# xxlong0/NeuralUDF

Hardware: NVIDIA H100
Metric: ray-samples/sec (render_core fwd+bwd) (higher is better)
Workload: dtype f32

## Files before the change

### neuraludf_b200/csrc/gemm_tc.cuh

```cuda
#pragma once
#include <cuda.h>
#include <cudaTypedefs.h>
#include <cuda_bf16.h>

#include "gemm_simt.cuh"

namespace nudf {
namespace tc {

constexpr int BM = 128;
constexpr int BN = 128;
constexpr int BK = 64;
constexpr int THREADS = 256;
constexpr int A_HALF_BYTES = BM * BK * 2;
constexpr int B_HALF_BYTES = BN * BK * 2;
__host__ __device__ constexpr int b_plane_bytes(int wn) { return wn * BK * 2; }
__host__ __device__ constexpr int acc_ld(int wn) { return wn + 4; }

__host__ __device__ inline int pad16(int n) { return (n + 15) & ~15; }
__host__ __device__ inline int pad64(int k) { return (k + 63) & ~63; }

__host__ __device__ inline uint32_t sw128(uint32_t row, uint32_t k) {
  return (row >> 3) * 1024u + (row & 7u) * 128u + ((((k >> 3) ^ (row & 7u)) & 7u) << 4) + ((k & 7u) << 1);
}

constexpr int TN_PS = 32;
constexpr int TN_RING = 4;
constexpr uint32_t TN_F32_OPND = TN_PS * BM * 4;
constexpr uint32_t TN_F32_STAGE = 2 * TN_F32_OPND;
constexpr uint32_t TN_PLANE = BM * TN_PS * 2;
constexpr uint32_t TN_PLANE_STAGE = 4 * TN_PLANE;
struct TnMaps { CUtensorMap a, b; };
__host__ __device__ inline uint32_t sw128_mn(uint32_t mn, uint32_t k) {
  return (mn >> 6) * 4096u + (k >> 3) * 1024u + (k & 7u) * 128u + ((((mn >> 3) ^ k) & 7u) << 4) + ((mn & 7u) << 1);
}

constexpr uint32_t W_SLOT = BM * BK * 4;
static_assert(W_SLOT == 2 * A_HALF_BYTES, "a slot holds exactly the two bf16 planes of its slice");
__host__ __device__ constexpr int w_ring(int wn) { return wn == 256 ? 3 : 4; }

__device__ __forceinline__ uint32_t pack_bf16(float a, float b) {
  __nv_bfloat162 v = __floats2bfloat162_rn(a, b);
  return *reinterpret_cast<uint32_t*>(&v);
}
template <int NP>
__device__ __forceinline__ void split4(const float x[4], uint2 planes[NP]) {
  float r[4] = {x[0], x[1], x[2], x[3]};
#pragma unroll
  for (int p = 0; p < NP; ++p) {
    float h[4];
#pragma unroll
    for (int j = 0; j < 4; ++j) {
      h[j] = __bfloat162float(__float2bfloat16_rn(r[j]));
      r[j] -= h[j];
    }
    planes[p] = make_uint2(pack_bf16(h[0], h[1]), pack_bf16(h[2], h[3]));
  }
}
__host__ __device__ inline int nt_of(int np) { return np == 2 ? 256 : 128; }
__host__ __device__ inline int n_tiles(int N, int np) { return (N + nt_of(np) - 1) / nt_of(np); }
__host__ __device__ inline int tile_rows(int N, int t, int np) { int r = N - nt_of(np) * t; return pad16(r < nt_of(np) ? r : nt_of(np)); }
__host__ __device__ inline int64_t tile_elems(int N, int K, int t, int np) { return (int64_t)(pad64(K) / 64) * np * tile_rows(N, t, np) * 64; }
__host__ __device__ inline int64_t tile_offset(int N, int K, int t, int np) {
  int64_t o = 0;
  for (int i = 0; i < t; ++i) o += tile_elems(N, K, i, np);
  return o;
}
__host__ __device__ inline int64_t image_elems(int N, int K, int np) { return tile_offset(N, K, n_tiles(N, np), np); }

static __device__ __forceinline__ void tc_prep_weights_body(const float* __restrict__ W, int64_t ldw, int N, int K, int transposed, int np,
                                                            uint16_t* __restrict__ img, int64_t start, int64_t stride) {
  const int Kp = pad64(K);
  const int nt = n_tiles(N, np);
  int64_t total = 0;
  for (int t = 0; t < nt; ++t) total += (int64_t)tile_rows(N, t, np) * Kp;
  for (int64_t idx = start; idx < total; idx += stride) {
    int64_t rem = idx;
    int t = 0;
    while (rem >= (int64_t)tile_rows(N, t, np) * Kp) { rem -= (int64_t)tile_rows(N, t, np) * Kp; ++t; }
    const int rows = tile_rows(N, t, np);
    const int nl = (int)(rem / Kp), k = (int)(rem - (int64_t)nl * Kp);
    const int n = t * nt_of(np) + nl;
    float x = 0.f;
    if (n < N && k < K) x = transposed ? W[(int64_t)k * ldw + n] : W[(int64_t)n * ldw + k];
    const int s = k >> 6, kl = k & 63;
    uint16_t* base = img + tile_offset(N, K, t, np) + (int64_t)s * np * rows * 64;
    const uint32_t off = sw128((uint32_t)nl, (uint32_t)kl) >> 1;
    float r = x;
    for (int p = 0; p < np; ++p) {
      __nv_bfloat16 h = __float2bfloat16_rn(r);
      base[(int64_t)p * rows * 64 + off] = __bfloat16_as_ushort(h);
      r -= __bfloat162float(h);
    }
  }
}
static __global__ void tc_prep_weights_kernel(const float* __restrict__ W, int64_t ldw, int N, int K, int transposed, int np,
                                              uint16_t* __restrict__ img) {
  tc_prep_weights_body(W, ldw, N, K, transposed, np, img, (int64_t)blockIdx.x * blockDim.x + threadIdx.x, (int64_t)gridDim.x * blockDim.x);
}


__device__ __forceinline__ uint32_t smem_u32(const void* p) { return (uint32_t)__cvta_generic_to_shared(p); }
__device__ __forceinline__ uint8_t* align1024(uint8_t* p) {
  return reinterpret_cast<uint8_t*>((reinterpret_cast<uintptr_t>(p) + 1023) & ~(uintptr_t)1023);
}

__device__ __forceinline__ void mbar_init(uint64_t* bar, uint32_t count) {
  asm volatile("mbarrier.init.shared::cta.b64 [%0], %1;" ::"r"(smem_u32(bar)), "r"(count) : "memory");
}
__device__ __forceinline__ void mbar_arrive_expect_tx(uint64_t* bar, uint32_t bytes) {
  asm volatile("mbarrier.arrive.expect_tx.shared::cta.b64 _, [%0], %1;" ::"r"(smem_u32(bar)), "r"(bytes) : "memory");
}
__device__ __forceinline__ uint32_t mbar_try_wait(uint32_t addr, uint32_t parity) {
  uint32_t ok;
  asm volatile(
      "{\n"
      ".reg .pred p;\n"
      "mbarrier.try_wait.parity.shared::cta.b64 p, [%1], %2;\n"
      "selp.u32 %0, 1, 0, p;\n"
      "}\n"
      : "=r"(ok)
      : "r"(addr), "r"(parity)
      : "memory");
  return ok;
}
__device__ __forceinline__ void mbar_wait(uint64_t* bar, uint32_t parity) {
  const uint32_t addr = smem_u32(bar);
  while (!mbar_try_wait(addr, parity)) {
  }
}
__device__ __forceinline__ void fence_barrier_init() { asm volatile("fence.mbarrier_init.release.cluster;" ::: "memory"); }
__device__ __forceinline__ void fence_proxy_async() { asm volatile("fence.proxy.async.shared::cta;" ::: "memory"); }

__device__ __forceinline__ void bulk_g2s(void* smem_dst, const void* gmem_src, uint32_t bytes, uint64_t* bar) {
  asm volatile("cp.async.bulk.shared::cluster.global.mbarrier::complete_tx::bytes [%0], [%1], %2, [%3];" ::"r"(smem_u32(smem_dst)),
               "l"(gmem_src), "r"(bytes), "r"(smem_u32(bar))
               : "memory");
}

__device__ __forceinline__ void tma_load_2d(void* smem_dst, const CUtensorMap* map, int c, int k, uint64_t* bar) {
  asm volatile("cp.async.bulk.tensor.2d.shared::cluster.global.mbarrier::complete_tx::bytes [%0], [%1, {%2, %3}], [%4];"
               ::"r"(smem_u32(smem_dst)), "l"(reinterpret_cast<uint64_t>(map)), "r"(c), "r"(k), "r"(smem_u32(bar))
               : "memory");
}

__device__ __forceinline__ uint64_t make_desc(uint32_t smem_addr) {
  return (uint64_t)((smem_addr & 0x3FFFFu) >> 4) | (1ull << 16) | (64ull << 32) | (1ull << 62);
}
__device__ __forceinline__ uint64_t make_desc_mn(uint32_t smem_addr) {
  return (uint64_t)((smem_addr & 0x3FFFFu) >> 4) | ((uint64_t)(4096 >> 4) << 16) | ((uint64_t)(1024 >> 4) << 32) | (1ull << 62);
}
__device__ __forceinline__ void wg_fence() { asm volatile("wgmma.fence.sync.aligned;" ::: "memory"); }
__device__ __forceinline__ void wg_commit() { asm volatile("wgmma.commit_group.sync.aligned;" ::: "memory"); }
__device__ __forceinline__ void wg_wait_all() { asm volatile("wgmma.wait_group.sync.aligned 0;" ::: "memory"); }
__device__ __forceinline__ void wg_wait_but_one() { asm volatile("wgmma.wait_group.sync.aligned 1;" ::: "memory"); }
template <int N>
__device__ __forceinline__ void fence_operand(float (&d)[N]) {
#pragma unroll
  for (int q = 0; q < N; ++q) asm volatile("" : "+f"(d[q])::"memory");
}
__device__ __forceinline__ float unbias_rz(float r) { return fmaf(__uint_as_float(__float_as_uint(r) & 0xff800000u), 0x1p-24f, r); }

template <int MN_MAJOR = 0>
__device__ __forceinline__ void wgmma_128(float (&d)[64], uint64_t da, uint64_t db, uint32_t accumulate) {
  asm volatile(
      "{\n"
      ".reg .pred p;\n"
      "setp.ne.b32 p, %66, 0;\n"
      "wgmma.mma_async.sync.aligned.m64n128k16.f32.bf16.bf16 "
      "{%0, %1, %2, %3, %4, %5, %6, %7, %8, %9, %10, %11, %12, %13, %14, %15, %16, %17, %18, %19, %20, %21, %22, %23, %24, %25, "
      "%26, %27, %28, %29, %30, %31, %32, %33, %34, %35, %36, %37, %38, %39, %40, %41, %42, %43, %44, %45, %46, %47, %48, %49, "
      "%50, %51, %52, %53, %54, %55, %56, %57, %58, %59, %60, %61, %62, %63}, %64, %65, p, 1, 1, %67, %67;\n"
      "}\n"
      : "+f"(d[0]), "+f"(d[1]), "+f"(d[2]), "+f"(d[3]), "+f"(d[4]), "+f"(d[5]), "+f"(d[6]), "+f"(d[7]), "+f"(d[8]), "+f"(d[9]),
        "+f"(d[10]), "+f"(d[11]), "+f"(d[12]), "+f"(d[13]), "+f"(d[14]), "+f"(d[15]), "+f"(d[16]), "+f"(d[17]), "+f"(d[18]),
        "+f"(d[19]), "+f"(d[20]), "+f"(d[21]), "+f"(d[22]), "+f"(d[23]), "+f"(d[24]), "+f"(d[25]), "+f"(d[26]), "+f"(d[27]),
        "+f"(d[28]), "+f"(d[29]), "+f"(d[30]), "+f"(d[31]), "+f"(d[32]), "+f"(d[33]), "+f"(d[34]), "+f"(d[35]), "+f"(d[36]),
        "+f"(d[37]), "+f"(d[38]), "+f"(d[39]), "+f"(d[40]), "+f"(d[41]), "+f"(d[42]), "+f"(d[43]), "+f"(d[44]), "+f"(d[45]),
        "+f"(d[46]), "+f"(d[47]), "+f"(d[48]), "+f"(d[49]), "+f"(d[50]), "+f"(d[51]), "+f"(d[52]), "+f"(d[53]), "+f"(d[54]),
        "+f"(d[55]), "+f"(d[56]), "+f"(d[57]), "+f"(d[58]), "+f"(d[59]), "+f"(d[60]), "+f"(d[61]), "+f"(d[62]), "+f"(d[63])
      : "l"(da), "l"(db), "r"(accumulate), "n"(MN_MAJOR));
}
__device__ __forceinline__ void wgmma_128_fresh(float (&d)[64], uint64_t da, uint64_t db) {
  asm volatile(
      "{\n"
      ".reg .pred p;\n"
      "setp.ne.b32 p, %66, 0;\n"
      "wgmma.mma_async.sync.aligned.m64n128k16.f32.bf16.bf16 "
      "{%0, %1, %2, %3, %4, %5, %6, %7, %8, %9, %10, %11, %12, %13, %14, %15, %16, %17, %18, %19, %20, %21, %22, %23, %24, %25, "
      "%26, %27, %28, %29, %30, %31, %32, %33, %34, %35, %36, %37, %38, %39, %40, %41, %42, %43, %44, %45, %46, %47, %48, %49, "
      "%50, %51, %52, %53, %54, %55, %56, %57, %58, %59, %60, %61, %62, %63}, %64, %65, p, 1, 1, 0, 0;\n"
      "}\n"
      : "=f"(d[0]), "=f"(d[1]), "=f"(d[2]), "=f"(d[3]), "=f"(d[4]), "=f"(d[5]), "=f"(d[6]), "=f"(d[7]), "=f"(d[8]), "=f"(d[9]),
        "=f"(d[10]), "=f"(d[11]), "=f"(d[12]), "=f"(d[13]), "=f"(d[14]), "=f"(d[15]), "=f"(d[16]), "=f"(d[17]), "=f"(d[18]),
        "=f"(d[19]), "=f"(d[20]), "=f"(d[21]), "=f"(d[22]), "=f"(d[23]), "=f"(d[24]), "=f"(d[25]), "=f"(d[26]), "=f"(d[27]),
        "=f"(d[28]), "=f"(d[29]), "=f"(d[30]), "=f"(d[31]), "=f"(d[32]), "=f"(d[33]), "=f"(d[34]), "=f"(d[35]), "=f"(d[36]),
        "=f"(d[37]), "=f"(d[38]), "=f"(d[39]), "=f"(d[40]), "=f"(d[41]), "=f"(d[42]), "=f"(d[43]), "=f"(d[44]), "=f"(d[45]),
        "=f"(d[46]), "=f"(d[47]), "=f"(d[48]), "=f"(d[49]), "=f"(d[50]), "=f"(d[51]), "=f"(d[52]), "=f"(d[53]), "=f"(d[54]),
        "=f"(d[55]), "=f"(d[56]), "=f"(d[57]), "=f"(d[58]), "=f"(d[59]), "=f"(d[60]), "=f"(d[61]), "=f"(d[62]), "=f"(d[63])
      : "l"(da), "l"(db), "r"(0u));
}

__device__ __forceinline__ void wgmma_256(float (&d)[128], uint64_t da, uint64_t db, uint32_t accumulate) {
  asm volatile(
      "{\n"
      ".reg .pred p;\n"
      "setp.ne.b32 p, %130, 0;\n"
      "wgmma.mma_async.sync.aligned.m64n256k16.f32.bf16.bf16 "
      "{%0, %1, %2, %3, %4, %5, %6, %7, %8, %9, %10, %11, %12, %13, %14, %15, %16, %17, %18, %19, %20, %21, %22, %23, %24, "
      "%25, %26, %27, %28, %29, %30, %31, %32, %33, %34, %35, %36, %37, %38, %39, %40, %41, %42, %43, %44, %45, %46, %47, "
      "%48, %49, %50, %51, %52, %53, %54, %55, %56, %57, %58, %59, %60, %61, %62, %63, %64, %65, %66, %67, %68, %69, %70, "
      "%71, %72, %73, %74, %75, %76, %77, %78, %79, %80, %81, %82, %83, %84, %85, %86, %87, %88, %89, %90, %91, %92, %93, "
      "%94, %95, %96, %97, %98, %99, %100, %101, %102, %103, %104, %105, %106, %107, %108, %109, %110, %111, %112, %113, "
      "%114, %115, %116, %117, %118, %119, %120, %121, %122, %123, %124, %125, %126, %127}, %128, %129, p, 1, 1, 0, 0;\n"
      "}\n"
      : "+f"(d[0]), "+f"(d[1]), "+f"(d[2]), "+f"(d[3]), "+f"(d[4]), "+f"(d[5]), "+f"(d[6]), "+f"(d[7]), "+f"(d[8]),
        "+f"(d[9]), "+f"(d[10]), "+f"(d[11]), "+f"(d[12]), "+f"(d[13]), "+f"(d[14]), "+f"(d[15]), "+f"(d[16]), "+f"(d[17]),
        "+f"(d[18]), "+f"(d[19]), "+f"(d[20]), "+f"(d[21]), "+f"(d[22]), "+f"(d[23]), "+f"(d[24]), "+f"(d[25]), "+f"(d[26]),
        "+f"(d[27]), "+f"(d[28]), "+f"(d[29]), "+f"(d[30]), "+f"(d[31]), "+f"(d[32]), "+f"(d[33]), "+f"(d[34]), "+f"(d[35]),
        "+f"(d[36]), "+f"(d[37]), "+f"(d[38]), "+f"(d[39]), "+f"(d[40]), "+f"(d[41]), "+f"(d[42]), "+f"(d[43]), "+f"(d[44]),
        "+f"(d[45]), "+f"(d[46]), "+f"(d[47]), "+f"(d[48]), "+f"(d[49]), "+f"(d[50]), "+f"(d[51]), "+f"(d[52]), "+f"(d[53]),
        "+f"(d[54]), "+f"(d[55]), "+f"(d[56]), "+f"(d[57]), "+f"(d[58]), "+f"(d[59]), "+f"(d[60]), "+f"(d[61]), "+f"(d[62]),
        "+f"(d[63]), "+f"(d[64]), "+f"(d[65]), "+f"(d[66]), "+f"(d[67]), "+f"(d[68]), "+f"(d[69]), "+f"(d[70]), "+f"(d[71]),
        "+f"(d[72]), "+f"(d[73]), "+f"(d[74]), "+f"(d[75]), "+f"(d[76]), "+f"(d[77]), "+f"(d[78]), "+f"(d[79]), "+f"(d[80]),
        "+f"(d[81]), "+f"(d[82]), "+f"(d[83]), "+f"(d[84]), "+f"(d[85]), "+f"(d[86]), "+f"(d[87]), "+f"(d[88]), "+f"(d[89]),
        "+f"(d[90]), "+f"(d[91]), "+f"(d[92]), "+f"(d[93]), "+f"(d[94]), "+f"(d[95]), "+f"(d[96]), "+f"(d[97]), "+f"(d[98]),
        "+f"(d[99]), "+f"(d[100]), "+f"(d[101]), "+f"(d[102]), "+f"(d[103]), "+f"(d[104]), "+f"(d[105]), "+f"(d[106]),
        "+f"(d[107]), "+f"(d[108]), "+f"(d[109]), "+f"(d[110]), "+f"(d[111]), "+f"(d[112]), "+f"(d[113]), "+f"(d[114]),
        "+f"(d[115]), "+f"(d[116]), "+f"(d[117]), "+f"(d[118]), "+f"(d[119]), "+f"(d[120]), "+f"(d[121]), "+f"(d[122]),
        "+f"(d[123]), "+f"(d[124]), "+f"(d[125]), "+f"(d[126]), "+f"(d[127])
      : "l"(da), "l"(db), "r"(accumulate));
}

template <int WN>
__device__ __forceinline__ void wgmma_n(float (&d)[WN / 2], uint64_t da, uint64_t db, uint32_t accumulate) {
  if constexpr (WN == 256) wgmma_256(d, da, db, accumulate);
  else wgmma_128(d, da, db, accumulate);
}
template <int NP, int WN>
__device__ __forceinline__ void mma_slice(float (&d)[WN / 2], uint32_t a, uint32_t a_stride, uint32_t b, uint32_t b_stride, bool zero_first) {
  auto desc = [](uint32_t base, uint32_t stride, int p, int j) { return make_desc(base + p * stride + 32u * j); };
#pragma unroll
  for (int j = 0; j < BK / 16; ++j) {
    const uint32_t acc0 = (zero_first && j == 0) ? 0u : 1u;
    if constexpr (NP == 2) {
      wgmma_n<WN>(d, desc(a, a_stride, 1, j), desc(b, b_stride, 0, j), acc0);
      wgmma_n<WN>(d, desc(a, a_stride, 0, j), desc(b, b_stride, 1, j), 1u);
      wgmma_n<WN>(d, desc(a, a_stride, 0, j), desc(b, b_stride, 0, j), 1u);
    } else {
      wgmma_n<WN>(d, desc(a, a_stride, 2, j), desc(b, b_stride, 0, j), acc0);
      wgmma_n<WN>(d, desc(a, a_stride, 0, j), desc(b, b_stride, 2, j), 1u);
      wgmma_n<WN>(d, desc(a, a_stride, 1, j), desc(b, b_stride, 1, j), 1u);
      wgmma_n<WN>(d, desc(a, a_stride, 1, j), desc(b, b_stride, 0, j), 1u);
      wgmma_n<WN>(d, desc(a, a_stride, 0, j), desc(b, b_stride, 1, j), 1u);
    }
  }
}
__device__ __forceinline__ void mma_slice_mn(float (&d)[64], uint32_t a, uint32_t b, bool zero_first) {
#pragma unroll
  for (int j = 0; j < TN_PS / 16; ++j) {
    const uint32_t acc0 = (zero_first && j == 0) ? 0u : 1u;
    const uint32_t aj = a + 2048u * j, bj = b + 2048u * j;
    wgmma_128<1>(d, make_desc_mn(aj + TN_PLANE), make_desc_mn(bj), acc0);
    wgmma_128<1>(d, make_desc_mn(aj), make_desc_mn(bj + TN_PLANE), 1u);
    wgmma_128<1>(d, make_desc_mn(aj), make_desc_mn(bj), 1u);
  }
}

template <int WN>
__device__ __forceinline__ void acc_to_smem(const float (&d)[WN / 2], float* acc_s, int wg, int wtid) {
  constexpr int LD = acc_ld(WN);
  const int r = 64 * wg + 16 * (wtid >> 5) + ((wtid & 31) >> 2);
  const int c = 2 * (wtid & 3);
#pragma unroll
  for (int g = 0; g < WN / 8; ++g) {
    *reinterpret_cast<float2*>(acc_s + r * LD + 8 * g + c) = make_float2(d[4 * g], d[4 * g + 1]);
    *reinterpret_cast<float2*>(acc_s + (r + 8) * LD + 8 * g + c) = make_float2(d[4 * g + 2], d[4 * g + 3]);
  }
}
template <class Epi> constexpr int epi_rows_in_flight() { return epi_family<Epi>::value == FAM_TC_OTHER ? 2 : 8; }
template <int WN, class Epi>
__device__ __forceinline__ void tile_epilogue(const float* acc_s, int64_t m0, int64_t M, int n0, int n_valid_end, const Epi& epi, int tid) {
  constexpr int LD = acc_ld(WN);
  constexpr int EPI_ROWS = epi_rows_in_flight<Epi>();
  const int cq = tid & 31;
#pragma unroll 1
  for (int h = 0; h < WN / 128; ++h) {
    const int cl = 128 * h + 4 * cq;
    const int col = n0 + cl;
    int nv = n_valid_end - col;
    nv = nv < 4 ? nv : 4;
    if (nv <= 0) break;
    for (int r0 = tid >> 5; r0 < BM; r0 += EPI_ROWS * (THREADS / 32)) {
      typename Epi::Aux aux[EPI_ROWS];
#pragma unroll
      for (int i = 0; i < EPI_ROWS; ++i) {
        const int64_t row = m0 + r0 + i * (THREADS / 32);
        if (row < M) epi.load(row, col, nv, aux[i]);
      }
#pragma unroll
      for (int i = 0; i < EPI_ROWS; ++i) {
        const int r = r0 + i * (THREADS / 32);
        const int64_t row = m0 + r;
        if (row < M) {
          const float4 t = *reinterpret_cast<const float4*>(acc_s + r * LD + cl);
          const float x[4] = {t.x, t.y, t.z, t.w};
          epi.apply(row, col, x, nv, aux[i]);
        }
      }
    }
  }
}

template <int NT>
__device__ __forceinline__ void fetch_a(const float* __restrict__ A, int64_t lda, int64_t m0, int64_t M, int k0, int K, int tid,
                                        bool vec_ok, float4 (&v)[BM * 16 / NT]) {
  const int c = tid & 15;
  const int rsub = tid >> 4;
  const int k = k0 + c * 4;
#pragma unroll
  for (int pass = 0; pass < BM * 16 / NT; ++pass) {
    const int64_t row = m0 + pass * (NT / 16) + rsub;
    v[pass] = make_float4(0.f, 0.f, 0.f, 0.f);
    if (row < M) {
      const float* p = A + row * lda + k;
      if (vec_ok && k + 3 < K) {
        v[pass] = *reinterpret_cast<const float4*>(p);
      } else {
        if (k + 0 < K) v[pass].x = p[0];
        if (k + 1 < K) v[pass].y = p[1];
        if (k + 2 < K) v[pass].z = p[2];
        if (k + 3 < K) v[pass].w = p[3];
      }
    }
  }
}
template <int NP, int NT>
__device__ __forceinline__ void store_a(const float4 (&v)[BM * 16 / NT], uint8_t* sa, int tid) {
  const int c = tid & 15;
  const int rsub = tid >> 4;
#pragma unroll
  for (int pass = 0; pass < BM * 16 / NT; ++pass) {
    const float x[4] = {v[pass].x, v[pass].y, v[pass].z, v[pass].w};
    uint2 pl[NP];
    split4<NP>(x, pl);
    const uint32_t off = sw128((uint32_t)(pass * (NT / 16) + rsub), (uint32_t)(c * 4));
#pragma unroll
    for (int p = 0; p < NP; ++p) *reinterpret_cast<uint2*>(sa + p * A_HALF_BYTES + off) = pl[p];
  }
}
template <int NP, int NT>
__device__ __forceinline__ void stage_a_direct(const float* __restrict__ A, int64_t lda, int64_t m0, int64_t M, int k0, int K,
                                               uint8_t* sa, int tid, bool vec_ok) {
  float4 v[BM * 16 / NT];
  fetch_a<NT>(A, lda, m0, M, k0, K, tid, vec_ok, v);
  store_a<NP, NT>(v, sa, tid);
}

__device__ __forceinline__ void fetch_block_t(const float* __restrict__ X, int64_t ld, int m0, int m_total, int r0, int rows,
                                              int64_t k0, int64_t k_end, int lane, bool vec_ok, float4 (&v)[8][2]) {
  const int mq = lane & 7, kq = lane >> 3;
  if (r0 + 4 * mq >= rows) return;
  const int m = m0 + r0 + 4 * mq;
#pragma unroll
  for (int q = 0; q < 8; ++q) {
#pragma unroll
    for (int kk = 0; kk < 2; ++kk) {
      const int64_t k = k0 + 2 * (4 * q + kq) + kk;
      v[q][kk] = make_float4(0.f, 0.f, 0.f, 0.f);
      if (k < k_end) {
        const float* p = X + k * ld + m;
        if (vec_ok && m + 3 < m_total) {
          v[q][kk] = *reinterpret_cast<const float4*>(p);
        } else {
          if (m + 0 < m_total) v[q][kk].x = p[0];
          if (m + 1 < m_total) v[q][kk].y = p[1];
          if (m + 2 < m_total) v[q][kk].z = p[2];
          if (m + 3 < m_total) v[q][kk].w = p[3];
        }
      }
    }
  }
}
template <bool CSUM = false>
__device__ __forceinline__ void store_block_t(const float4 (&v)[8][2], int r0, int rows, uint8_t* s_hi, uint8_t* s_lo, int lane,
                                              float* csum = nullptr) {
  const int mq = lane & 7, kq = lane >> 3;
  if (r0 + 4 * mq >= rows) return;
  if (CSUM) {
#pragma unroll
    for (int q = 0; q < 8; ++q) {
      csum[0] += v[q][0].x + v[q][1].x; csum[1] += v[q][0].y + v[q][1].y;
      csum[2] += v[q][0].z + v[q][1].z; csum[3] += v[q][0].w + v[q][1].w;
    }
  }
#pragma unroll
  for (int q = 0; q < 8; ++q) {
    const float x0[4] = {v[q][0].x, v[q][0].y, v[q][0].z, v[q][0].w};
    const float x1[4] = {v[q][1].x, v[q][1].y, v[q][1].z, v[q][1].w};
#pragma unroll
    for (int j = 0; j < 4; ++j) {
      const float h0 = __bfloat162float(__float2bfloat16_rn(x0[j])), h1 = __bfloat162float(__float2bfloat16_rn(x1[j]));
      const uint32_t off = sw128((uint32_t)(r0 + 4 * mq + j), (uint32_t)(2 * (4 * q + kq)));
      *reinterpret_cast<uint32_t*>(s_hi + off) = pack_bf16(h0, h1);
      *reinterpret_cast<uint32_t*>(s_lo + off) = pack_bf16(x0[j] - h0, x1[j] - h1);
    }
  }
}

template <int NP, int WN, class Epi, bool RING>
__global__ void __launch_bounds__(THREADS, 1)
gemm_w_kernel(const float* __restrict__ A, int64_t lda, int64_t M, int N, int K, const uint16_t* __restrict__ img, Epi epi,
              const __grid_constant__ CUtensorMap amap) {
  static_assert(WN == 128 || (WN == 256 && NP == 2), "WN = 256 only with 2 planes (3 planes need 2 x WN/2 accumulators)");
  static_assert(!RING || NP == 2, "the ring path splits a slot into 2 planes in place");
  extern __shared__ uint8_t smem_raw[];
  uint8_t* smem = align1024(smem_raw);
  const int tid = threadIdx.x, wg = tid >> 7;
  const int n_ct = (N + WN - 1) / WN;
  const int n0 = (int)(blockIdx.x % (unsigned)n_ct) * WN;
  const int64_t m0 = (int64_t)(blockIdx.x / (unsigned)n_ct) * BM;
  const int t = n0 / nt_of(NP);
  const int rows_t = tile_rows(N, t, NP);
  const int row_in_tile = n0 - t * nt_of(NP);
  int rows_h = rows_t - row_in_tile; rows_h = rows_h < WN ? rows_h : WN;
  const int n_slices = pad64(K) / 64;
  constexpr uint32_t B_PLANE = b_plane_bytes(WN);
  const uint16_t* img_t = img + tile_offset(N, K, t, NP) + (int64_t)row_in_tile * 64;
  constexpr int NACC = WN / 2, NTOT = NP == 3 ? 64 : 1;
  float acc[NACC], tot[NTOT], acc2[NTOT];
#pragma unroll
  for (int q = 0; q < NACC; ++q) acc[q] = 0.f;
#pragma unroll
  for (int q = 0; q < NTOT; ++q) tot[q] = 0.f;

  if constexpr (RING) {
    constexpr int NR = w_ring(WN);
    constexpr uint32_t W_STAGE = 2 * B_PLANE;
    uint8_t* wst = smem + NR * W_SLOT;
    uint64_t* afull = reinterpret_cast<uint64_t*>(wst + 2 * W_STAGE);
    uint64_t* wfull = afull + NR;
    auto issue_a = [&](int i) {
      const int r = i % NR;
      mbar_arrive_expect_tx(&afull[r], W_SLOT);
      tma_load_2d(smem + r * W_SLOT, &amap, i * BK, (int)m0, &afull[r]);
    };
    auto issue_w = [&](int ks) {
      uint8_t* st = wst + (ks & 1) * W_STAGE;
      const uint32_t wb = (uint32_t)rows_h * 128u;
      mbar_arrive_expect_tx(&wfull[ks & 1], 2 * wb);
      for (int p = 0; p < 2; ++p) bulk_g2s(st + p * B_PLANE, img_t + ((int64_t)ks * 2 + p) * rows_t * 64, wb, &wfull[ks & 1]);
    };
    auto split = [&](int i) {
      uint8_t* slot = smem + (i % NR) * W_SLOT;
      mbar_wait(&afull[i % NR], (uint32_t)((i / NR) & 1));
      float4 v[BM * 16 / THREADS];
      const float4* f = reinterpret_cast<const float4*>(slot) + (tid >> 4) * (BK / 4) + (tid & 15);
#pragma unroll
      for (int pass = 0; pass < BM * 16 / THREADS; ++pass) v[pass] = f[pass * (THREADS / 16) * (BK / 4)];
      __syncthreads();
      store_a<2, THREADS>(v, slot, tid);
    };
    if (tid == 0) {
      for (int r = 0; r < NR; ++r) mbar_init(&afull[r], 1);
      mbar_init(&wfull[0], 1);
      mbar_init(&wfull[1], 1);
      fence_barrier_init();
      if (n_slices > 0) issue_w(0);
      for (int i = 0; i < NR && i < n_slices; ++i) issue_a(i);
    }
    __syncthreads();
    if (n_slices > 0) {
      split(0);
      fence_proxy_async();
    }
    __syncthreads();
    for (int ks = 0; ks < n_slices; ++ks) {
      const int s = ks & 1;
      if (tid == 0 && ks + 1 < n_slices) issue_w(ks + 1);
      mbar_wait(&wfull[s], (uint32_t)((ks >> 1) & 1));
      const uint32_t sa = smem_u32(smem + (ks % NR) * W_SLOT), sb = smem_u32(wst + s * W_STAGE);
      wg_fence();
      mma_slice<2, WN>(acc, sa + wg * (64 * 128), A_HALF_BYTES, sb, B_PLANE, ks == 0);
      wg_commit();
      if (ks + 1 < n_slices) split(ks + 1);
      wg_wait_all();
      fence_proxy_async();
      __syncthreads();
      if (tid == 0 && ks + NR < n_slices) issue_a(ks + NR);
    }
  } else {
    const uint32_t a_bytes = NP * A_HALF_BYTES, stage_bytes = a_bytes + NP * B_PLANE;
    uint64_t* full = reinterpret_cast<uint64_t*>(smem + 2 * stage_bytes);
    const bool vec_ok = ((lda & 3) == 0) && aligned16(A);

    auto issue_copies = [&](int ks) {
      uint8_t* st = smem + (ks & 1) * stage_bytes;
      const uint32_t wb = (uint32_t)rows_h * 128u;
      mbar_arrive_expect_tx(&full[ks & 1], NP * wb);
      for (int p = 0; p < NP; ++p) bulk_g2s(st + a_bytes + p * B_PLANE, img_t + ((int64_t)ks * NP + p) * rows_t * 64, wb, &full[ks & 1]);
    };
    if (tid == 0) {
      mbar_init(&full[0], 1);
      mbar_init(&full[1], 1);
      fence_barrier_init();
    }
    __syncthreads();
    if (n_slices > 0) {
      if (tid == 0) issue_copies(0);
      stage_a_direct<NP, THREADS>(A, lda, m0, M, 0, K, smem, tid, vec_ok);
      fence_proxy_async();
    }
    __syncthreads();
    for (int ks = 0; ks < n_slices; ++ks) {
      const int s = ks & 1;
      if (tid == 0 && ks + 1 < n_slices) issue_copies(ks + 1);
      mbar_wait(&full[s], (uint32_t)((ks >> 1) & 1));
      const uint32_t st = smem_u32(smem + s * stage_bytes);
      wg_fence();
      mma_slice<NP, WN>(acc, st + wg * (64 * 128), A_HALF_BYTES, st + a_bytes, B_PLANE, NP == 3 || ks == 0);
      wg_commit();
      if (ks + 1 < n_slices) stage_a_direct<NP, THREADS>(A, lda, m0, M, (ks + 1) * BK, K, smem + (s ^ 1) * stage_bytes, tid, vec_ok);
      wg_wait_all();
      if constexpr (NP == 3) {
        static_assert(BK / 16 == 4, "four hi * hi steps per K slice");
        auto hi_hi = [&](float (&d)[64], int j) {
          wg_fence();
          wgmma_128_fresh(d, make_desc(st + wg * (64 * 128) + 32u * j), make_desc(st + a_bytes + 32u * j));
          wg_commit();
        };
        auto add_unbiased = [&](float (&d)[64]) {
          fence_operand(d);
#pragma unroll
          for (int q = 0; q < 64; ++q) tot[q] += unbias_rz(d[q]);
        };
        hi_hi(acc2, 0);
        fence_operand(acc);
#pragma unroll
        for (int q = 0; q < 64; ++q) tot[q] += acc[q];
        hi_hi(acc, 1);
        wg_wait_but_one();
        add_unbiased(acc2);
        hi_hi(acc2, 2);
        wg_wait_but_one();
        add_unbiased(acc);
        hi_hi(acc, 3);
        wg_wait_but_one();
        add_unbiased(acc2);
        wg_wait_all();
        add_unbiased(acc);
      }
      fence_proxy_async();
      __syncthreads();
    }
  }
  float* acc_s = reinterpret_cast<float*>(smem);
  if constexpr (NP == 3) acc_to_smem<WN>(tot, acc_s, wg, tid & 127);
  else acc_to_smem<WN>(acc, acc_s, wg, tid & 127);
  __syncthreads();
  tile_epilogue<WN>(acc_s, m0, M, n0, N, epi, tid);
}

template <class Epi, bool RING>
__global__ void __launch_bounds__(THREADS, 1)
gemm_tn_kernel(const float* __restrict__ A, int64_t lda, const float* __restrict__ B, int64_t ldb, int M, int N, int64_t K, int64_t k_chunk,
               Epi epi, float* __restrict__ colsum, float* __restrict__ cs_ws, const __grid_constant__ TnMaps maps) {
  extern __shared__ uint8_t smem_raw[];
  uint8_t* smem = align1024(smem_raw);
  const int tid = threadIdx.x, wg = tid >> 7, warp = tid >> 5, lane = tid & 31;
  const int m0 = blockIdx.x * BM;
  const int n0 = blockIdx.y * BN;
  const int64_t kb = (int64_t)blockIdx.z * k_chunk;
  const int64_t ke = (kb + k_chunk < K) ? kb + k_chunk : K;
  const bool do_csum = colsum != nullptr && blockIdx.y == 0;
  float csum[4] = {0.f, 0.f, 0.f, 0.f};
  if (ke <= kb) return;
  float acc[64];
#pragma unroll
  for (int q = 0; q < 64; ++q) acc[q] = 0.f;
  if constexpr (RING) {
    uint8_t* ring = smem;
    uint8_t* planes = smem + TN_RING * TN_F32_STAGE;
    float* cs_part = reinterpret_cast<float*>(planes + 2 * TN_PLANE_STAGE);
    uint64_t* full = reinterpret_cast<uint64_t*>(cs_part + 4 * BM);
    const int n_sl = (int)((ke - kb + TN_PS - 1) / TN_PS);
    const int opnd = warp >> 2, kq = warp & 3;

    auto issue = [&](int i) {
      const int r = i % TN_RING;
      const int k0 = (int)(kb + (int64_t)i * TN_PS);
      uint8_t* st = ring + r * TN_F32_STAGE;
      mbar_arrive_expect_tx(&full[r], TN_F32_STAGE);
      tma_load_2d(st, &maps.a, m0, k0, &full[r]);
      tma_load_2d(st + TN_F32_OPND, &maps.b, n0, k0, &full[r]);
    };
    auto split = [&](int i, uint8_t* dst) {
      const int r = i % TN_RING;
      mbar_wait(&full[r], (uint32_t)((i / TN_RING) & 1));
      const float* f = reinterpret_cast<const float*>(ring + r * TN_F32_STAGE + opnd * TN_F32_OPND) + 4 * lane;
      uint8_t* hi = dst + opnd * 2 * TN_PLANE;
      const int64_t k0 = kb + (int64_t)i * TN_PS;
#pragma unroll
      for (int q = 0; q < TN_PS / 8; ++q) {
        float4 v[2];
#pragma unroll
        for (int kk = 0; kk < 2; ++kk) {
          const int p = 8 * q + 2 * kq + kk;
          v[kk] = k0 + p < ke ? *reinterpret_cast<const float4*>(f + p * BM) : make_float4(0.f, 0.f, 0.f, 0.f);
        }
        if (opnd == 0 && do_csum) {
          csum[0] += v[0].x + v[1].x; csum[1] += v[0].y + v[1].y;
          csum[2] += v[0].z + v[1].z; csum[3] += v[0].w + v[1].w;
        }
#pragma unroll
        for (int kk = 0; kk < 2; ++kk) {
          const float x[4] = {v[kk].x, v[kk].y, v[kk].z, v[kk].w};
          uint2 pl[2];
          split4<2>(x, pl);
          const uint32_t off = sw128_mn(4u * lane, (uint32_t)(8 * q + 2 * kq + kk));
          *reinterpret_cast<uint2*>(hi + off) = pl[0];
          *reinterpret_cast<uint2*>(hi + TN_PLANE + off) = pl[1];
        }
      }
    };
    if (tid == 0) {
      for (int r = 0; r < TN_RING; ++r) mbar_init(&full[r], 1);
      fence_barrier_init();
      for (int i = 0; i < TN_RING && i < n_sl; ++i) issue(i);
    }
    __syncthreads();
    split(0, planes);
    fence_proxy_async();
    __syncthreads();
    if (tid == 0 && TN_RING < n_sl) issue(TN_RING);
    for (int i = 0; i < n_sl; ++i) {
      const int s = i & 1;
      const uint32_t st = smem_u32(planes + s * TN_PLANE_STAGE);
      wg_fence();
      mma_slice_mn(acc, st + wg * 4096u, st + 2 * TN_PLANE, i == 0);
      wg_commit();
      if (i + 1 < n_sl) split(i + 1, planes + (s ^ 1) * TN_PLANE_STAGE);
      wg_wait_all();
      fence_proxy_async();
      __syncthreads();
      if (tid == 0 && i + 1 + TN_RING < n_sl) issue(i + 1 + TN_RING);
    }
    if (do_csum && opnd == 0)
#pragma unroll
      for (int j = 0; j < 4; ++j) cs_part[kq * BM + 4 * lane + j] = csum[j];
  } else {
    int rows_b = N - n0; rows_b = pad16(rows_b < BN ? rows_b : BN);
    const int n_sl = (int)((ke - kb + BK - 1) / BK);
    constexpr uint32_t stage_bytes = 2u * A_HALF_BYTES + 2u * B_HALF_BYTES;
    const bool a_vec = ((lda & 3) == 0) && aligned16(A) && ((m0 & 3) == 0);
    const bool b_vec = ((ldb & 3) == 0) && aligned16(B);
    const bool b_warp = warp >= 4 && 32 * (warp - 4) < rows_b;
    float4 v[8][2];

    auto fetch = [&](int i) {
      const int64_t k0 = kb + (int64_t)i * BK;
      if (warp < 4) fetch_block_t(A, lda, m0, M, 32 * warp, BM, k0, ke, lane, a_vec, v);
      else if (b_warp) fetch_block_t(B, ldb, n0, N, 32 * (warp - 4), rows_b, k0, ke, lane, b_vec, v);
    };
    auto store = [&](uint8_t* st) {
      if (warp < 4) {
        if (do_csum) store_block_t<true>(v, 32 * warp, BM, st, st + A_HALF_BYTES, lane, csum);
        else store_block_t(v, 32 * warp, BM, st, st + A_HALF_BYTES, lane);
      } else if (b_warp) {
        store_block_t(v, 32 * (warp - 4), rows_b, st + 2 * A_HALF_BYTES, st + 2 * A_HALF_BYTES + B_HALF_BYTES, lane);
      }
    };
    fetch(0);
    store(smem);
    if (n_sl > 1) fetch(1);
    fence_proxy_async();
    __syncthreads();
    for (int i = 0; i < n_sl; ++i) {
      const int s = i & 1;
      const uint32_t st = smem_u32(smem + s * stage_bytes);
      wg_fence();
      mma_slice<2, BN>(acc, st + wg * (64 * 128), A_HALF_BYTES, st + 2 * A_HALF_BYTES, B_HALF_BYTES, i == 0);
      wg_commit();
      if (i + 1 < n_sl) {
        store(smem + (s ^ 1) * stage_bytes);
        if (i + 2 < n_sl) fetch(i + 2);
      }
      wg_wait_all();
      fence_proxy_async();
      __syncthreads();
    }
    if (do_csum && warp < 4) {
#pragma unroll
      for (int j = 0; j < 4; ++j) {
        csum[j] += __shfl_xor_sync(0xffffffffu, csum[j], 8);
        csum[j] += __shfl_xor_sync(0xffffffffu, csum[j], 16);
      }
      const int m = m0 + 32 * warp + 4 * (lane & 7);
      if ((lane >> 3) == 0)
#pragma unroll
        for (int j = 0; j < 4; ++j)
          if (m + j < M) {
            if (cs_ws != nullptr) cs_ws[(int64_t)blockIdx.z * M + m + j] = csum[j];
            else colsum[m + j] += csum[j];
          }
    }
  }
  float* acc_s = reinterpret_cast<float*>(smem);
  acc_to_smem<BN>(acc, acc_s, wg, tid & 127);
  __syncthreads();
  if constexpr (RING) {
    const float* cs_part = reinterpret_cast<const float*>(smem + TN_RING * TN_F32_STAGE + 2 * TN_PLANE_STAGE);
    if (do_csum && tid < BM && m0 + tid < M) {
      const float c = (cs_part[tid] + cs_part[BM + tid]) + (cs_part[2 * BM + tid] + cs_part[3 * BM + tid]);
      if (cs_ws != nullptr) cs_ws[(int64_t)blockIdx.z * M + m0 + tid] = c;
      else colsum[m0 + tid] += c;
    }
  }
  tile_epilogue<BN>(acc_s, m0, M, n0, N, epi, tid);
}

static inline int sm_count() {
  static int n = 0;
  if (n == 0) {
    int dev = 0;
    if (cudaGetDevice(&dev) != cudaSuccess || cudaDeviceGetAttribute(&n, cudaDevAttrMultiProcessorCount, dev) != cudaSuccess || n <= 0) n = 132;
  }
  return n;
}


static inline int tensor_map_2d(CUtensorMap* map, const float* X, int64_t ld, int64_t cols, int64_t rows, int box_cols, int box_rows) {
  static PFN_cuTensorMapEncodeTiled encode = nullptr;
  if (encode == nullptr) {
    void* fn = nullptr;
    cudaDriverEntryPointQueryResult q;
    if (cudaGetDriverEntryPoint("cuTensorMapEncodeTiled", &fn, cudaEnableDefault, &q) != cudaSuccess || q != cudaDriverEntryPointSuccess ||
        fn == nullptr) {
      nudf::set_error("cuTensorMapEncodeTiled is not available from the driver");
      return -2;
    }
    encode = reinterpret_cast<PFN_cuTensorMapEncodeTiled>(fn);
  }
  const cuuint64_t dims[2] = {(cuuint64_t)cols, (cuuint64_t)rows};
  const cuuint64_t strides[1] = {(cuuint64_t)ld * sizeof(float)};
  const cuuint32_t box[2] = {(cuuint32_t)box_cols, (cuuint32_t)box_rows};
  const cuuint32_t elem[2] = {1, 1};
  const CUresult r = encode(map, CU_TENSOR_MAP_DATA_TYPE_FLOAT32, 2, const_cast<float*>(X), dims, strides, box, elem,
                            CU_TENSOR_MAP_INTERLEAVE_NONE, CU_TENSOR_MAP_SWIZZLE_NONE, CU_TENSOR_MAP_L2_PROMOTION_L2_256B,
                            CU_TENSOR_MAP_FLOAT_OOB_FILL_NONE);
  if (r != CUDA_SUCCESS) {
    nudf::set_error("cuTensorMapEncodeTiled failed (%d)", (int)r);
    return -2;
  }
  return 0;
}
constexpr size_t w_smem_bytes(int np, int wn) { return 2 * (size_t)np * (A_HALF_BYTES + b_plane_bytes(wn)) + 2 * sizeof(uint64_t) + 1024; }
static_assert(BM * acc_ld(2 * BN) * sizeof(float) <= 2 * 2 * (size_t)(A_HALF_BYTES + b_plane_bytes(2 * BN)), "accumulator tile");
constexpr size_t w_ring_operand_bytes(int wn) { return (size_t)w_ring(wn) * W_SLOT + 2 * 2 * (size_t)b_plane_bytes(wn); }
constexpr size_t w_ring_smem_bytes(int wn) { return w_ring_operand_bytes(wn) + (w_ring(wn) + 2) * sizeof(uint64_t) + 1024; }
static_assert(w_ring_smem_bytes(BN) <= 227 * 1024 && w_ring_smem_bytes(2 * BN) <= 227 * 1024, "one CTA per SM");
static_assert(BM * acc_ld(BN) * sizeof(float) <= w_ring_operand_bytes(BN), "accumulator tile in the ring path's stages");
static_assert(BM * acc_ld(2 * BN) * sizeof(float) <= w_ring_operand_bytes(2 * BN), "accumulator tile in the ring path's stages");

template <int NP, int WN, class Epi, bool RING>
static inline int gemm_w_launch(const float* A, int64_t lda, int64_t M, int N, int K, const uint16_t* img, const Epi& epi, cudaStream_t st) {
  constexpr size_t smem = RING ? w_ring_smem_bytes(WN) : w_smem_bytes(NP, WN);
  static bool attr_set = false;
  if (!attr_set) {
    NUDF_CUDA_OK(cudaFuncSetAttribute(gemm_w_kernel<NP, WN, Epi, RING>, cudaFuncAttributeMaxDynamicSharedMemorySize, (int)smem));
    attr_set = true;
  }
  CUtensorMap amap{};
  if constexpr (RING)
    if (int rc = tensor_map_2d(&amap, A, lda, K, M, BK, BM)) return rc;
  const unsigned grid = (unsigned)(cdiv(M, BM) * cdiv(N, WN));
  LaunchTimer lt_(epi_family<Epi>::value, st);
  gemm_w_kernel<NP, WN, Epi, RING><<<grid, THREADS, smem, st>>>(A, lda, M, N, K, img, epi, amap);
  NUDF_LAUNCH_OK();
  return 0;
}
template <int NP, int WN, class Epi>
static inline int gemm_w_path(const float* A, int64_t lda, int64_t M, int N, int K, const uint16_t* img, const Epi& epi, cudaStream_t st) {
  if constexpr (NP == 2)
    if (K > 0 && (lda & 3) == 0 && aligned16(A)) return gemm_w_launch<2, WN, Epi, true>(A, lda, M, N, K, img, epi, st);
  return gemm_w_launch<NP, WN, Epi, false>(A, lda, M, N, K, img, epi, st);
}
template <int NP, class Epi>
static inline int gemm_w(const float* A, int64_t lda, int64_t M, int N, int K, const uint16_t* img, const Epi& epi, cudaStream_t st) {
  if (M <= 0 || N <= 0) return 0;
  if constexpr (NP == 2)
    if (N > BN) return gemm_w_path<2, 2 * BN, Epi>(A, lda, M, N, K, img, epi, st);
  return gemm_w_path<NP, BN, Epi>(A, lda, M, N, K, img, epi, st);
}

constexpr int TN_WAVE_CTAS = 132;
constexpr int64_t TN_MIN_POINTS = 512;
static inline int64_t tn_k_chunk(int M, int N, int64_t K) {
  const int64_t tiles = cdiv(M, BM) * cdiv(N, BN);
  int64_t splits = TN_WAVE_CTAS / tiles;
  if (splits > cdiv(K, TN_MIN_POINTS)) splits = cdiv(K, TN_MIN_POINTS);
  splits = ws_splits(splits < 1 ? 1 : (int)splits, (int64_t)M * N + M);
  return round_up(cdiv(K, splits), BK);
}

constexpr size_t TN_SMEM = 2 * (size_t)(2 * A_HALF_BYTES + 2 * B_HALF_BYTES) + 2 * sizeof(uint64_t) + 1024;
constexpr size_t TN_RING_SMEM = (size_t)TN_RING * TN_F32_STAGE + 2 * TN_PLANE_STAGE + 4 * BM * sizeof(float) + TN_RING * sizeof(uint64_t) + 1024;
static_assert(BM * acc_ld(BN) * sizeof(float) <= (size_t)TN_RING * TN_F32_STAGE, "accumulator tile in the ring");
static_assert(TN_RING_SMEM <= 227 * 1024, "one CTA per SM");

template <class Epi, bool RING>
static inline int gemm_tn_launch(dim3 grid, const float* A, int64_t lda, const float* B, int64_t ldb, int M, int N, int64_t K,
                                 int64_t k_chunk, const Epi& epi, float* colsum, float* cs_ws, cudaStream_t st) {
  constexpr size_t smem = RING ? TN_RING_SMEM : TN_SMEM;
  static bool attr_set = false;
  if (!attr_set) {
    NUDF_CUDA_OK(cudaFuncSetAttribute(gemm_tn_kernel<Epi, RING>, cudaFuncAttributeMaxDynamicSharedMemorySize, (int)smem));
    attr_set = true;
  }
  TnMaps maps{};
  if constexpr (RING) {
    if (int rc = tensor_map_2d(&maps.a, A, lda, M, K, BM, TN_PS)) return rc;
    if (int rc = tensor_map_2d(&maps.b, B, ldb, N, K, BN, TN_PS)) return rc;
  }
  gemm_tn_kernel<Epi, RING><<<grid, THREADS, smem, st>>>(A, lda, B, ldb, M, N, K, k_chunk, epi, colsum, cs_ws, maps);
  NUDF_LAUNCH_OK();
  return 0;
}
template <class Epi>
static inline int gemm_tn(const float* A, int64_t lda, const float* B, int64_t ldb, int M, int N, int64_t K, const Epi& epi,
                          cudaStream_t st, float* colsum_a = nullptr) {
  if (M <= 0 || N <= 0 || K <= 0) return 0;
  const int64_t k_chunk = tn_k_chunk(M, N, K);
  const int splits = (int)cdiv(K, k_chunk);
  dim3 grid((unsigned)cdiv(M, BM), (unsigned)cdiv(N, BN), (unsigned)splits);
  LaunchTimer lt_(FAM_TC_WGRAD, st);
  const bool ring = (lda & 3) == 0 && (ldb & 3) == 0 && aligned16(A) && aligned16(B);
  if (splits == 1) {
    if (ring) return gemm_tn_launch<Epi, true>(grid, A, lda, B, ldb, M, N, K, k_chunk, epi, colsum_a, nullptr, st);
    return gemm_tn_launch<Epi, false>(grid, A, lda, B, ldb, M, N, K, k_chunk, epi, colsum_a, nullptr, st);
  }
  float* ws = split_workspace(st);
  if (ws == nullptr) return -2;
  float* cs = ws + (int64_t)splits * M * N;
  const EpiSplitStore e{ws, (int64_t)M * N, N};
  if (int rc = ring ? gemm_tn_launch<EpiSplitStore, true>(grid, A, lda, B, ldb, M, N, K, k_chunk, e, colsum_a, cs, st)
                    : gemm_tn_launch<EpiSplitStore, false>(grid, A, lda, B, ldb, M, N, K, k_chunk, e, colsum_a, cs, st))
    return rc;
  if (int rc = splitk_reduce(ws, splits, M, N, epi, st)) return rc;
  return colsum_a != nullptr ? vec_reduce(cs, splits, M, colsum_a, st) : 0;
}

struct PrepWJob { const float* W; uint16_t* img; int ldw, N, K, transposed, np; };
struct PrepWJobs { int n; PrepWJob j[64]; };
static __global__ void tc_prep_weights_jobs_kernel(const __grid_constant__ PrepWJobs jobs) {
  const PrepWJob& J = jobs.j[blockIdx.y];
  tc_prep_weights_body(J.W, J.ldw, J.N, J.K, J.transposed, J.np, J.img, (int64_t)blockIdx.x * blockDim.x + threadIdx.x,
                       (int64_t)gridDim.x * blockDim.x);
}
static inline int prep_weights_jobs(const PrepWJobs& jobs, cudaStream_t st) {
  if (jobs.n <= 0) return 0;
  int64_t mx = 0;
  for (int i = 0; i < jobs.n; ++i) {
    int64_t total = 0;
    for (int t = 0; t < n_tiles(jobs.j[i].N, jobs.j[i].np); ++t) total += (int64_t)tile_rows(jobs.j[i].N, t, jobs.j[i].np) * pad64(jobs.j[i].K);
    mx = total > mx ? total : mx;
  }
  int blocks = (int)((mx + 255) / 256);
  if (blocks > 1024) blocks = 1024;
  tc_prep_weights_jobs_kernel<<<dim3((unsigned)blocks, (unsigned)jobs.n), 256, 0, st>>>(jobs);
  NUDF_LAUNCH_OK();
  return 0;
}

static inline int prep_weights(const float* W, int64_t ldw, int N, int K, int transposed, int np, uint16_t* img, cudaStream_t st) {
  int64_t total = 0;
  for (int t = 0; t < n_tiles(N, np); ++t) total += (int64_t)tile_rows(N, t, np) * pad64(K);
  int blocks = (int)((total + 255) / 256);
  if (blocks > 4096) blocks = 4096;
  tc_prep_weights_kernel<<<blocks, 256, 0, st>>>(W, ldw, N, K, transposed, np, img);
  NUDF_LAUNCH_OK();
  return 0;
}

}
}
```

Before: 7.557 million.

## Add warp-specialized persistent TMA kernel for three-plane bf16 weight GEMM

Adds a persistent 384-thread kernel for the three-plane (NP==3) weight GEMM path. One producer warpgroup streams fp32 A in quarter-tile TMA loads, splits it into bf16 planes in shared memory, and bulk-copies the weight planes, all behind full/empty mbarriers. Two consumer warpgroups run wgmma with registers rebalanced through setmaxnreg. The epilogue now runs straight from registers instead of staging through shared memory. split4 is also simplified to reuse the packed bf16 bits for the residual, which removes the round-trip conversions.

```diff
diff --git a/neuraludf_b200/csrc/gemm_tc.cuh b/neuraludf_b200/csrc/gemm_tc.cuh
--- a/neuraludf_b200/csrc/gemm_tc.cuh
+++ b/neuraludf_b200/csrc/gemm_tc.cuh
@@ -48,13 +48,12 @@
   float r[4] = {x[0], x[1], x[2], x[3]};
 #pragma unroll
   for (int p = 0; p < NP; ++p) {
-    float h[4];
-#pragma unroll
-    for (int j = 0; j < 4; ++j) {
-      h[j] = __bfloat162float(__float2bfloat16_rn(r[j]));
-      r[j] -= h[j];
-    }
-    planes[p] = make_uint2(pack_bf16(h[0], h[1]), pack_bf16(h[2], h[3]));
+    const uint32_t a = pack_bf16(r[0], r[1]), b = pack_bf16(r[2], r[3]);
+    planes[p] = make_uint2(a, b);
+    r[0] -= __uint_as_float(a << 16);
+    r[1] -= __uint_as_float(a & 0xffff0000u);
+    r[2] -= __uint_as_float(b << 16);
+    r[3] -= __uint_as_float(b & 0xffff0000u);
   }
 }
 __host__ __device__ inline int nt_of(int np) { return np == 2 ? 256 : 128; }
@@ -108,6 +107,9 @@
 __device__ __forceinline__ void mbar_init(uint64_t* bar, uint32_t count) {
   asm volatile("mbarrier.init.shared::cta.b64 [%0], %1;" ::"r"(smem_u32(bar)), "r"(count) : "memory");
 }
+__device__ __forceinline__ void mbar_arrive(uint64_t* bar) {
+  asm volatile("mbarrier.arrive.shared::cta.b64 _, [%0];" ::"r"(smem_u32(bar)) : "memory");
+}
 __device__ __forceinline__ void mbar_arrive_expect_tx(uint64_t* bar, uint32_t bytes) {
   asm volatile("mbarrier.arrive.expect_tx.shared::cta.b64 _, [%0], %1;" ::"r"(smem_u32(bar)), "r"(bytes) : "memory");
 }
@@ -150,6 +152,9 @@
 __device__ __forceinline__ uint64_t make_desc_mn(uint32_t smem_addr) {
   return (uint64_t)((smem_addr & 0x3FFFFu) >> 4) | ((uint64_t)(4096 >> 4) << 16) | ((uint64_t)(1024 >> 4) << 32) | (1ull << 62);
 }
+__device__ __forceinline__ void wg_bar_sync() { asm volatile("bar.sync 1, 128;" ::: "memory"); }
+template <uint32_t R> __device__ __forceinline__ void reg_dealloc() { asm volatile("setmaxnreg.dec.sync.aligned.u32 %0;" ::"n"(R)); }
+template <uint32_t R> __device__ __forceinline__ void reg_alloc() { asm volatile("setmaxnreg.inc.sync.aligned.u32 %0;" ::"n"(R)); }
 __device__ __forceinline__ void wg_fence() { asm volatile("wgmma.fence.sync.aligned;" ::: "memory"); }
 __device__ __forceinline__ void wg_commit() { asm volatile("wgmma.commit_group.sync.aligned;" ::: "memory"); }
 __device__ __forceinline__ void wg_wait_all() { asm volatile("wgmma.wait_group.sync.aligned 0;" ::: "memory"); }
@@ -561,6 +566,173 @@
   tile_epilogue<WN>(acc_s, m0, M, n0, N, epi, tid);
 }
 
+constexpr int W3_THREADS = 384;
+constexpr int W3_QROWS = 32;
+constexpr uint32_t W3_QUARTER = W3_QROWS * BK * 4;
+constexpr int W3_NQ = BM / W3_QROWS;
+constexpr uint32_t W3_A_STAGE = 3 * A_HALF_BYTES;
+constexpr uint32_t W3_STAGE = W3_A_STAGE + 3 * b_plane_bytes(BN);
+constexpr uint32_t W3_LAND = W3_NQ * W3_QUARTER;
+constexpr int W3_PRODUCER_REGS = 40, W3_CONSUMER_REGS = 232;
+static_assert(W3_LAND == W_SLOT, "the landing quarters hold one fp32 slice");
+static_assert(W3_PRODUCER_REGS + 2 * W3_CONSUMER_REGS <= 65536 / 128, "register file of one SM");
+static_assert(BM * 16 / 128 / W3_NQ == 4, "four float4 per producer thread and quarter");
+
+template <class Epi>
+__global__ void __launch_bounds__(W3_THREADS, 1)
+gemm_w3_tma_kernel(const float* __restrict__ A, int64_t M, int N, int K, const uint16_t* __restrict__ img, Epi epi,
+                   const __grid_constant__ CUtensorMap amap) {
+  extern __shared__ uint8_t smem_raw[];
+  uint8_t* smem = align1024(smem_raw);
+  uint8_t* land = smem + 2 * W3_STAGE;
+  uint64_t* full = reinterpret_cast<uint64_t*>(land + W3_LAND);
+  uint64_t* empty = full + 2;
+  uint64_t* landed = empty + 2;
+  const int tid = threadIdx.x, wg = tid >> 7;
+  const int n_ct = (N + BN - 1) / BN;
+  const int tiles = (int)((M + BM - 1) / BM) * n_ct;
+  const int n_slices = pad64(K) / 64;
+  constexpr uint32_t B_PLANE = b_plane_bytes(BN);
+  if (tid == 0) {
+    mbar_init(&full[0], 129);
+    mbar_init(&full[1], 129);
+    mbar_init(&empty[0], 256);
+    mbar_init(&empty[1], 256);
+    for (int q = 0; q < W3_NQ; ++q) mbar_init(&landed[q], 1);
+    fence_barrier_init();
+  }
+  __syncthreads();
+
+  if (wg == 0) {
+    reg_dealloc<W3_PRODUCER_REGS>();
+    auto issue_quarter = [&](int t, int ks, int q) {
+      const int64_t r0 = (int64_t)(t / n_ct) * BM + q * W3_QROWS;
+      if (r0 < M) {
+        mbar_arrive_expect_tx(&landed[q], W3_QUARTER);
+        tma_load_2d(land + q * W3_QUARTER, &amap, ks * BK, (int)r0, &landed[q]);
+      } else {
+        mbar_arrive(&landed[q]);
+      }
+    };
+    if (tid == 0 && (int)blockIdx.x < tiles)
+      for (int q = 0; q < W3_NQ; ++q) issue_quarter(blockIdx.x, 0, q);
+    const int c = tid & 15, rsub = tid >> 4;
+    uint32_t g = 0;
+    for (int t = blockIdx.x; t < tiles; t += gridDim.x) {
+      const int64_t m0 = (int64_t)(t / n_ct) * BM;
+      const int tn = t % n_ct;
+      const int rows_t = tile_rows(N, tn, 3);
+      const uint16_t* img_t = img + tile_offset(N, K, tn, 3);
+      for (int ks = 0; ks < n_slices; ++ks, ++g) {
+        int t1 = t, ks1 = ks + 1;
+        if (ks1 == n_slices) { ks1 = 0; t1 += gridDim.x; }
+        const int s = g & 1;
+        uint8_t* st = smem + s * W3_STAGE;
+        mbar_wait(&empty[s], ((g >> 1) & 1) ^ 1);
+        if (tid == 0) {
+          const uint32_t wb = (uint32_t)rows_t * 128u;
+          mbar_arrive_expect_tx(&full[s], 3 * wb);
+          for (int p = 0; p < 3; ++p) bulk_g2s(st + W3_A_STAGE + p * B_PLANE, img_t + ((int64_t)ks * 3 + p) * rows_t * 64, wb, &full[s]);
+        }
+#pragma unroll 1
+        for (int q = 0; q < W3_NQ; ++q) {
+          float4 v[4];
+          if (m0 + q * W3_QROWS < M) {
+            mbar_wait(&landed[q], g & 1);
+            const float4* f = reinterpret_cast<const float4*>(land + q * W3_QUARTER) + rsub * (BK / 4) + c;
+#pragma unroll
+            for (int pass = 0; pass < 4; ++pass) v[pass] = f[pass * 8 * (BK / 4)];
+          } else {
+#pragma unroll
+            for (int pass = 0; pass < 4; ++pass) v[pass] = make_float4(0.f, 0.f, 0.f, 0.f);
+          }
+#pragma unroll
+          for (int pass = 0; pass < 4; ++pass) {
+            const float x[4] = {v[pass].x, v[pass].y, v[pass].z, v[pass].w};
+            uint2 pl[3];
+            split4<3>(x, pl);
+            const uint32_t off = sw128((uint32_t)(q * W3_QROWS + pass * 8 + rsub), (uint32_t)(c * 4));
+#pragma unroll
+            for (int p = 0; p < 3; ++p) *reinterpret_cast<uint2*>(st + p * A_HALF_BYTES + off) = pl[p];
+          }
+          fence_proxy_async();
+          wg_bar_sync();
+          if (tid == 0 && t1 < tiles) issue_quarter(t1, ks1, q);
+        }
+        fence_proxy_async();
+        mbar_arrive(&full[s]);
+      }
+    }
+  } else {
+    reg_alloc<W3_CONSUMER_REGS>();
+    const int cw = wg - 1, wtid = tid & 127, lane = tid & 31;
+    float acc[64], acc2[64], tot[64];
+    auto hi_hi = [&](float (&d)[64], uint32_t a, uint32_t b, int j) {
+      wg_fence();
+      wgmma_128_fresh(d, make_desc(a + 32u * j), make_desc(b + 32u * j));
+      wg_commit();
+    };
+    auto add_unbiased = [&](float (&d)[64]) {
+      fence_operand(d);
+#pragma unroll
+      for (int q = 0; q < 64; ++q) tot[q] += unbias_rz(d[q]);
+    };
+    uint32_t g = 0;
+    for (int t = blockIdx.x; t < tiles; t += gridDim.x) {
+      const int64_t m0 = (int64_t)(t / n_ct) * BM;
+      const int n0 = (t % n_ct) * BN;
+#pragma unroll
+      for (int q = 0; q < 64; ++q) tot[q] = 0.f;
+      for (int ks = 0; ks < n_slices; ++ks, ++g) {
+        const int s = g & 1;
+        mbar_wait(&full[s], (g >> 1) & 1);
+        const uint32_t a = smem_u32(smem + s * W3_STAGE) + cw * (64 * 128), b = smem_u32(smem + s * W3_STAGE + W3_A_STAGE);
+        wg_fence();
+        mma_slice<3, BN>(acc, a, A_HALF_BYTES, b, B_PLANE, true);
+        wg_commit();
+        hi_hi(acc2, a, b, 0);
+        wg_wait_but_one();
+        fence_operand(acc);
+#pragma unroll
+        for (int q = 0; q < 64; ++q) tot[q] += acc[q];
+        hi_hi(acc, a, b, 1);
+        wg_wait_but_one();
+        add_unbiased(acc2);
+        hi_hi(acc2, a, b, 2);
+        wg_wait_but_one();
+        add_unbiased(acc);
+        hi_hi(acc, a, b, 3);
+        wg_wait_but_one();
+        add_unbiased(acc2);
+        wg_wait_all();
+        mbar_arrive(&empty[s]);
+        add_unbiased(acc);
+      }
+      const bool odd = lane & 1;
+      const int64_t row = m0 + 64 * cw + 16 * (wtid >> 5) + (lane >> 2) + (odd ? 8 : 0);
+      const int cbase = n0 + 4 * ((lane & 3) >> 1);
+      constexpr int EPI_G = sizeof(typename Epi::Aux) <= 4 * sizeof(float) ? 8 : 4;
+#pragma unroll
+      for (int j0 = 0; j0 < 16; j0 += EPI_G) {
+        typename Epi::Aux aux[EPI_G];
+#pragma unroll
+        for (int i = 0; i < EPI_G; ++i) {
+          const int col = cbase + 8 * (j0 + i);
+          if (row < M && col < N) epi.load(row, col, N - col < 4 ? N - col : 4, aux[i]);
+        }
+#pragma unroll
+        for (int i = 0; i < EPI_G; ++i) {
+          const int j = j0 + i, col = cbase + 8 * j;
+          const float s0 = odd ? tot[4 * j] : tot[4 * j + 2], s1 = odd ? tot[4 * j + 1] : tot[4 * j + 3];
+          const float r0 = __shfl_xor_sync(0xffffffffu, s0, 1), r1 = __shfl_xor_sync(0xffffffffu, s1, 1);
+          const float x[4] = {odd ? r0 : tot[4 * j], odd ? r1 : tot[4 * j + 1], odd ? tot[4 * j + 2] : r0, odd ? tot[4 * j + 3] : r1};
+          if (row < M && col < N) epi.apply(row, col, x, N - col < 4 ? N - col : 4, aux[i]);
+        }
+      }
+    }
+  }
+}
+
 template <class Epi, bool RING>
 __global__ void __launch_bounds__(THREADS, 1)
 gemm_tn_kernel(const float* __restrict__ A, int64_t lda, const float* __restrict__ B, int64_t ldb, int M, int N, int64_t K, int64_t k_chunk,
@@ -779,10 +951,31 @@
   NUDF_LAUNCH_OK();
   return 0;
 }
+constexpr size_t W3_SMEM = 2 * (size_t)W3_STAGE + W3_LAND + 8 * sizeof(uint64_t) + 1024;
+static_assert(W3_SMEM <= 227 * 1024, "one CTA per SM");
+
+template <class Epi>
+static inline int gemm_w3_tma_launch(const float* A, int64_t lda, int64_t M, int N, int K, const uint16_t* img, const Epi& epi, cudaStream_t st) {
+  static bool attr_set = false;
+  if (!attr_set) {
+    NUDF_CUDA_OK(cudaFuncSetAttribute(gemm_w3_tma_kernel<Epi>, cudaFuncAttributeMaxDynamicSharedMemorySize, (int)W3_SMEM));
+    attr_set = true;
+  }
+  CUtensorMap amap{};
+  if (int rc = tensor_map_2d(&amap, A, lda, K, M, BK, W3_QROWS)) return rc;
+  const int64_t tiles = cdiv(M, BM) * cdiv(N, BN);
+  const unsigned grid = (unsigned)(tiles < sm_count() ? tiles : sm_count());
+  LaunchTimer lt_(epi_family<Epi>::value, st);
+  gemm_w3_tma_kernel<Epi><<<grid, W3_THREADS, W3_SMEM, st>>>(A, M, N, K, img, epi, amap);
+  NUDF_LAUNCH_OK();
+  return 0;
+}
 template <int NP, int WN, class Epi>
 static inline int gemm_w_path(const float* A, int64_t lda, int64_t M, int N, int K, const uint16_t* img, const Epi& epi, cudaStream_t st) {
-  if constexpr (NP == 2)
-    if (K > 0 && (lda & 3) == 0 && aligned16(A)) return gemm_w_launch<2, WN, Epi, true>(A, lda, M, N, K, img, epi, st);
+  if (K > 0 && (lda & 3) == 0 && aligned16(A)) {
+    if constexpr (NP == 2) return gemm_w_launch<2, WN, Epi, true>(A, lda, M, N, K, img, epi, st);
+    else return gemm_w3_tma_launch<Epi>(A, lda, M, N, K, img, epi, st);
+  }
   return gemm_w_launch<NP, WN, Epi, false>(A, lda, M, N, K, img, epi, st);
 }
 template <int NP, class Epi>
```

Result: faster. 8.056 million (median of 6 runs) (+6.6%).
